# multiplefish/VPLines-SLAM

Measured on AMD Instinct MI355X. Metric: sliding-window BA solves/sec (10 KF, 200 pts + 80 lines, 5 iters), higher is better.
Workload: dtype f64

## Files before the change

vplines-slam_amd/csrc/ba_step.h:

```cpp
#pragma once
#include "ba_common.h"
#include "ba_solve.h"

namespace vpl {

constexpr int SCHUR_THREADS = 256;
constexpr int CHOL_THREADS = 256;
constexpr int BACK_THREADS = 256;

__device__ __forceinline__ void lds_ticket_wait(int* t, int seq) {
  while (__hip_atomic_load(t, __ATOMIC_RELAXED, __HIP_MEMORY_SCOPE_WORKGROUP) != seq) __builtin_amdgcn_s_sleep(1);
  __builtin_amdgcn_fence(__ATOMIC_ACQUIRE, "workgroup", "local");
}
__device__ __forceinline__ void lds_ticket_pass(int* t, int seq, int lane) {
  __builtin_amdgcn_fence(__ATOMIC_RELEASE, "workgroup", "local");
  if (lane == 0) __hip_atomic_store(t, seq + 1, __ATOMIC_RELAXED, __HIP_MEMORY_SCOPE_WORKGROUP);
}

__device__ __forceinline__ int compact2vis(int c, int s, int WS) {
  if (c < WS - 6) { const int v = 6 * s + c; return v < 66 ? v : -1; }
  if (c < WS) return 66 + (c - (WS - 6));
  return c < WS + 2 ? 72 + (c - WS) : -1;
}

// ... 287 lines not shown
      for (int b = 0; b < 4; ++b) if (b <= a) {
        A[t] = s4[a] * s4[b] * Hl[4 * a + b];
        if (a == b) A[t] += mu * d4[a] * d4[a];
        ++t;
      }
    bool ok = true;
    chol4(A, ok);
    if (!ok) flag[0] = 1;
    double us[4];
#pragma unroll
    for (int k = 0; k < 10; ++k) { lch[l * 10 + k] = A[k]; lC[l * 10 + k] = A[k]; }
#pragma unroll
    for (int a = 0; a < 4; ++a) {
      const double rd = 1.0 / A[tri(a, a)];
      lS[4 * l + a] = s4[a] * rd;
      us[a] = g4[a] / d4[a];
#pragma unroll
      for (int qd = 0; qd < 4; ++qd) if (qd < a) lC[l * 10 + tri(a, qd)] = A[tri(a, qd)] * rd;
    }
#pragma unroll
    for (int a = 0; a < 4; ++a) {
      double s2 = 0;
#pragma unroll
      for (int qd = 0; qd < 4; ++qd) if (qd >= a) s2 += A[tri(qd, a)] * us[qd];
      lE[4 * l + a] = s2;
    }
    {
      double xg[4];
#pragma unroll
      for (int a = 0; a < 4; ++a) {
        double s2 = (s4[a] / A[tri(a, a)]) * (g4[a] * d4[a] / s4[a]);
#pragma unroll
        for (int qd = 0; qd < 4; ++qd) if (qd < a) s2 -= (A[tri(a, qd)] / A[tri(a, a)]) * xg[qd];
        xg[a] = s2;
        lG[4 * l + a] = s2;
      }
    }
  }
  __syncthreads();
  for (int i = tid; i < CSQ_N; i += T) Cacc[i] = 0.0;
  for (int i = tid; i < NLT * 4 * 64; i += T) {
    const int ln = i & 63, v = (i >> 6) & 3, t = i >> 8;
    int ta = 0, tb = 0;
    tri_decode(t, ta, tb);
    const int ca = 16 * ta + (ln >> 4) + 4 * v, cb = 16 * tb + (ln & 15);
    int code = -1;
    if (ca >= cb && ca < WSv + 2 && cb < WSv) {
      const int a0 = compact2vis(ca, 0, WSv), b0 = compact2vis(cb, 0, WSv);
      const int step = (ca < WSv - 6 ? CSQ_LD : 0) + (cb < WSv - 6 ? 1 : 0);
      code = (a0 * CSQ_LD + b0) | step << 16;
    }
    ftab[i] = code;
  }
  __syncthreads();
  VPL_STAMP(B, w, 2);
  {
    const int m = lane & 15, kk = lane >> 4;
    const int wrow = lane < SK_WSTRIDE ? B.sk_wave[((size_t)w * 8 + wv) * SK_WSTRIDE + lane] : -1;
    const int nchunk = __builtin_amdgcn_readlane(wrow, 0);
    auto fetch = [&](int k) {
      int4 e = etab[k];
      e.x = __builtin_amdgcn_readfirstlane(e.x); e.y = __builtin_amdgcn_readfirstlane(e.y); e.z = __builtin_amdgcn_readfirstlane(e.z);
      return e;
    };
    v4d acc[NLT];
#pragma unroll
    for (int t = 0; t < NLT; ++t) acc[t] = v4d{0, 0, 0, 0};
    const double* Wp = B.Wp + (size_t)w * B.maxP * WS;
    const double* Wl = B.Wl + (size_t)w * B.maxL * 4 * WS;
    const double* gpv = B.gp + (size_t)w * B.maxP;
    const double* glv = B.gl + (size_t)w * B.maxL * 4;
    double wm[NTC], gm[NTC], em[NTC];
    int cl[NTC];
#pragma unroll
    for (int t = 0; t < NTC; ++t) {
      const int c = 16 * t + m;
      wm[t] = c < WSv ? 1.0 : 0.0;
      gm[t] = c == WSv ? 1.0 : 0.0;
      em[t] = c == WSv + 1 ? 1.0 : 0.0;
      cl[t] = c < WSv - 6 ? c : (c < WSv ? c + coff : WS - 1);
    }
    auto lm_id = [&](const int4 e) { return ((kk & 2 ? e.z : e.y) >> (16 * (kk & 1))) & 0xffff; };
    auto load_raw = [&](const int4 e, double (&raw)[NTC][4]) {
      const bool isl = (e.x & 32) != 0;
      const int idr = lm_id(e);
      const int id = idr != 0xffff ? idr : 0;
      if (isl) {
        const double* Wr = Wl + (unsigned)(id * 4 * WS);
#pragma unroll
        for (int t = 0; t < NTC; ++t)
#pragma unroll
          for (int qd = 0; qd < 4; ++qd) raw[t][qd] = Wr[(unsigned)(qd * WS + cl[t])];
      } else {
#pragma unroll
        for (int t = 0; t < NTC; ++t) raw[t][0] = Wp[(unsigned)(id * WS + cl[t])];
#pragma unroll
        for (int t = 0; t < NTC; ++t)
#pragma unroll
          for (int qd = 1; qd < 4; ++qd) raw[t][qd] = 0.0;
      }
    };
    auto transform = [&](const int4 e, const double (&raw)[NTC][4], double (&x)[NTC][4]) {
      const bool isl = (e.x & 32) != 0;
      const int idr = lm_id(e);
      const int id = idr != 0xffff ? idr : 0;
      const double pm = idr != 0xffff ? 1.0 : 0.0;
      if (isl) {
        const double* C = lC + id * 10;
        const double s0 = lS[4 * id] * pm, s1 = lS[4 * id + 1] * pm, s2 = lS[4 * id + 2] * pm, s3 = lS[4 * id + 3] * pm;
        const double c10 = C[1], c20 = C[3], c21 = C[4], c30 = C[6], c31 = C[7], c32 = C[8];
        double ev[4], gv[4];
#pragma unroll
        for (int a = 0; a < 4; ++a) { ev[a] = lE[4 * id + a] * pm; gv[a] = lG[4 * id + a] * pm; }
#pragma unroll
        for (int t = 0; t < NTC; ++t) {
          const double x0 = s0 * raw[t][0];
          const double x1 = s1 * raw[t][1] - c10 * x0;
          const double x2 = s2 * raw[t][2] - c20 * x0 - c21 * x1;
          const double x3 = s3 * raw[t][3] - c30 * x0 - c31 * x1 - c32 * x2;
          x[t][0] = x0 * wm[t] + gv[0] * gm[t] + ev[0] * em[t];
          x[t][1] = x1 * wm[t] + gv[1] * gm[t] + ev[1] * em[t];
          x[t][2] = x2 * wm[t] + gv[2] * gm[t] + ev[2] * em[t];
          x[t][3] = x3 * wm[t] + gv[3] * gm[t] + ev[3] * em[t];
        }
      } else {
        const double sp = pS[id] * pm, ep = pE[id] * pm, gq = pG[id] * pm;
#pragma unroll
        for (int t = 0; t < NTC; ++t) {
          x[t][0] = sp * raw[t][0] * wm[t] + gq * gm[t] + ep * em[t];
          x[t][1] = 0.0; x[t][2] = 0.0; x[t][3] = 0.0;
        }
      }
    };
#ifdef VPL_STAMPS
    long long st_flush = 0, st_wait = 0, st_xf = 0, st_mf = 0, st_ld = 0;
#endif
    auto flush = [&](int g, int seq) {
#ifdef VPL_STAMPS
      const long long tf0 = __builtin_readcyclecounter();
#endif
      const int s6 = 6 * (g & 15);
      int code[NLT * 4];
#pragma unroll
      for (int i = 0; i < NLT * 4; ++i) code[i] = ftab[i * 64 + lane];
      lds_ticket_wait(&tick[0], seq);
#ifdef VPL_STAMPS
      st_wait += __builtin_readcyclecounter() - tf0;
#endif
#pragma unroll
      for (int t = 0; t < NLT; ++t) {
        const double vals[4] = {acc[t].x, acc[t].y, acc[t].z, acc[t].w};
#pragma unroll
        for (int v = 0; v < 4; ++v) {
          const int c2 = code[4 * t + v];
          if (c2 >= 0) lds_add(&Cacc[(c2 & 0xffff) + s6 * (c2 >> 16)], vals[v]);
        }
        acc[t] = v4d{0, 0, 0, 0};
      }
      lds_ticket_pass(&tick[0], seq, lane);
#ifdef VPL_STAMPS
      st_flush += __builtin_readcyclecounter() - tf0;
#endif
    };
    int nent = 0;
#pragma unroll 1
    for (int ch = 0; ch < nchunk; ++ch) {
      const int k0 = __builtin_amdgcn_readlane(wrow, __builtin_amdgcn_readfirstlane(1 + 3 * ch));
      const int k1 = __builtin_amdgcn_readlane(wrow, __builtin_amdgcn_readfirstlane(2 + 3 * ch));
      const int seq = __builtin_amdgcn_readlane(wrow, __builtin_amdgcn_readfirstlane(3 + 3 * ch));
      nent += k1 - k0;
      if (MIXED && (fetch(k0).x & 64)) {
        SchurWide A;
        A.etab = etab; A.Wp = Wp; A.Wl = Wl; A.WS = WS; A.lC = lC; A.lS = lS; A.lE = lE; A.lG = lG; A.pS = pS; A.pE = pE; A.pG = pG;
        A.Cacc = Cacc; A.tick = tick;
        schur_wide_chunk(A, k0, k1, seq);
        continue;
      }
      double raw0[NTC][4], raw1[NTC][4], raw2[NTC][4];
      constexpr int NPF = 3;
      load_raw(fetch(k0), raw0);
      load_raw(fetch(min(k0 + 1, k1 - 1)), raw1);
      load_raw(fetch(min(k0 + 2, k1 - 1)), raw2);
      const int gcur = fetch(k0).x;
      auto step = [&](int k, double (&rw)[NTC][4]) {
        const int4 e = fetch(k);
#ifdef VPL_STAMPS
        const long long ts0 = __builtin_readcyclecounter();
#endif
        double x[NTC][4];
        transform(e, rw, x);
#ifdef VPL_STAMPS
        const long long ts1 = __builtin_readcyclecounter();
        st_xf += ts1 - ts0;
#endif
        load_raw(fetch(min(k + NPF, k1 - 1)), rw);
#ifdef VPL_STAMPS
        const long long ts2 = __builtin_readcyclecounter();
        st_ld += ts2 - ts1;
#endif
        const bool isl = (e.x & 32) != 0;
#pragma unroll
        for (int a = 0; a < 4; ++a) {
          if (a == 0 || isl) {
            int t = 0;
#pragma unroll
            for (int ta = 0; ta < NTC; ++ta)
#pragma unroll
              for (int tb = 0; tb <= ta; ++tb, ++t) acc[t] = __builtin_amdgcn_mfma_f64_16x16x4f64(x[ta][a], x[tb][a], acc[t], 0, 0, 0);
          }
        }
#ifdef VPL_STAMPS
        st_mf += __builtin_readcyclecounter() - ts2;
#endif
      };
#pragma unroll 1
      for (int kb = k0; kb < k1; kb += NPF) {
        step(kb, raw0);
        if (kb + 1 < k1) step(kb + 1, raw1);
        if (kb + 2 < k1) step(kb + 2, raw2);
      }
      flush(gcur, seq);
    }
#ifdef VPL_STAMPS
    if (lane == 0 && wv < 2) {
      long long* dg_ = B.dbg + (size_t)w * 64 + 30 + 6 * wv;
      dg_[0] = st_xf; dg_[1] = st_ld; dg_[2] = st_mf; dg_[3] = st_flush; dg_[4] = st_wait; dg_[5] = nent;
    }
#endif
  }
  __syncthreads();
  VPL_STAMP(B, w, 3);
  for (int b = tid; b < NV; b += T) qq += 2.0 * Cacc[(NV + 1) * CSQ_LD + b] * uc[vis2cam(b)];
  double* sacc = B.sacc + (size_t)w * SACC_N;
  for (int i = tid; i < SACC_N; i += T) {
    int a, b;
    tri_decode(i, a, b);
    sacc[i] = Cacc[a * CSQ_LD + b];
  }
  a1 = block_sum(a1, red);
  q = block_sum(q, red);
  qq = block_sum(qq, red);
  if (tid == 0) {
    tr->a1 = a1;
    tr->alpha = a1 / (q + qq);
    if (flag[0]) B.path[w] = 2;
  }
  VPL_STAMP(B, w, 4);
}

template <int NTC>
__global__ __launch_bounds__(SCHUR_THREADS, 2) void k_schur(DevBatch B) {
  extern __shared__ double sm[];
  if (blockIdx.x == 0 && threadIdx.x == 0) { B.ord_cnt[2 * ((B.ord_it + 1) & 1)] = 0; B.ord_cnt[2 * ((B.ord_it + 1) & 1) + 1] = 0; }
  schur_body<NTC>(B, ordered_window(B), sm);
}
__global__ __launch_bounds__(SCHUR_THREADS, 2) void k_schur_mixed(DevBatch B) {
  extern __shared__ double sm[];
  if (blockIdx.x == 0 && threadIdx.x == 0) { B.ord_cnt[2 * ((B.ord_it + 1) & 1)] = 0; B.ord_cnt[2 * ((B.ord_it + 1) & 1) + 1] = 0; }
  schur_body<3, true>(B, ordered_window(B), sm);
}
inline size_t schur_smem(int maxP, int maxL, int ntc = 5) {
  const int r1 = std::max(4 * maxP + 28 * maxL, (int)CSQ_N);
  const int maxKS = maxP / 4 + maxL + NF + 2;
  return (size_t)(r1 + 3 * maxP + 22 * maxL + 176 + 24) * sizeof(double) + (size_t)(8 + 4 * maxKS + ntc * (ntc + 1) / 2 * 256) * sizeof(int);
}

constexpr int DN = 90;
constexpr int DNT = 6;
constexpr int DNAP = DNT * (DNT + 1) / 2 * 256;
#ifdef VPL_CHOL_OCC3
constexpr int XLD = 66;
constexpr int CHOL_MIN_WAVES = 3;
#else
constexpr int XLD = 72;
constexpr int CHOL_MIN_WAVES = 2;
#endif
constexpr int XROWS_A = 36, XROWS_B = 48;

__device__ __forceinline__ int chain_frame(int ch, int b) { return ch == 0 ? 1 + b : 10 - b; }
__device__ __forceinline__ int chain_col(int ch, int b, int lane) {
  if (lane < 18) {
    const int ds = (b & 1) ? 9 : 0;
    const int f = chain_frame(ch, b);
    const int fr = (lane >= ds && lane < ds + 9) ? f : (ch == 0 ? f + 1 : f - 1);
    return 15 * fr + 6 + (lane < 9 ? lane : lane - 9);
  }
  if (ch == 0) {
    if (lane < 27) return 6 + (lane - 18);
    if (lane < 63) return 15 * ((lane - 27) / 6) + (lane - 27) % 6;
    return NC;
  }
  if (lane < 54) return 15 * (5 + (lane - 18) / 6) + (lane - 18) % 6;
  return lane == 54 ? NC : -1;
}
__device__ __forceinline__ int cam2dense(int c) {
  if (c < 0) return -1;
  if (c == NC) return DN;
  const int v = cam2vis(c);
  if (v >= 0) return v;
  if (c < 15) return 72 + (c - 6);
  return (c >= 81 && c < 90) ? c : -1;
}
__device__ __forceinline__ int dense2cam(int d) { return d < NV ? vis2cam(d) : (d < 81 ? 6 + (d - 72) : d); }
__device__ __forceinline__ int chain_dense(int ch, int lane) {
  if (lane < 18) {
    const bool s5 = ch == 0 ? lane < 9 : lane >= 9;
    return s5 ? 81 + (lane < 9 ? lane : lane - 9) : -1;
  }
  return cam2dense(chain_col(ch, 0, lane));
}

__device__ __forceinline__ void chol_body(const DevBatch& B, const int w, double* sm) {
  const int tid = threadIdx.x, T = CHOL_THREADS;
  const int lane = tid & 63, wv = ((tid >> 6) + ((blockIdx.x >> 8) & 1) * 2) & 3;
  TrState* tr = &B.tr[w];
  if (tr->status != 0 || tr->reuse != 0 || B.path[w] != 0) return;
  count_active(B, 1);
  constexpr int REG = (XROWS_A + XROWS_B) * XLD > DNAP ? (XROWS_A + XROWS_B) * XLD : DNAP;
  double* XA = sm;
  double* XBm = sm + XROWS_A * XLD;
  double* S = sm;
  double* scv = sm + REG;
  double* dgv = scv + 176;
  double* ycam = dgv + 176;
  double* yv = ycam + 176;
  double* isd = yv + 96;
  double* Linv = isd + 96;
  double* red = Linv + 256;
  int* flag = (int*)(red + 24);
  int* cdmap = flag + 8;
  double* rsL = (double*)(cdmap + 128);

  const size_t fb = (size_t)w * B.nfull;
  const double* gscale = B.scale + fb;
  const double* gdiag = B.diag + fb;
  const double* ggrad = B.grad + fb;
  double* ggn = B.gn + fb;
  const double* Hcc = B.Hcc + (size_t)w * NCP;
  const double* gc = B.gc + (size_t)w * NC;
  const double* sacc = B.sacc + (size_t)w * SACC_N;
  const double mu = tr->mu;
  for (int c = tid; c < 176; c += T) { scv[c] = c < NC ? gscale[c] : 0.0; dgv[c] = c < NC ? gdiag[c] : 1.0; ycam[c] = 0.0; }
  if (tid < 4) flag[tid] = 0;
  if (tid < 128) cdmap[tid] = chain_dense(tid >> 6, tid & 63);
  for (int i = tid; i < 3 * XLD; i += T) XBm[(XROWS_B - 3) * XLD + i] = 0.0;
  __syncthreads();
  VPL_STAMP(B, w, 8);

  double U[45];
#pragma unroll
  for (int i = 0; i < 45; ++i) U[i] = 0.0;
#define Xs(b, k) U[9 * (b) + (k)]
  if (wv < 2) {
    const int ch = wv, nblk = ch == 0 ? 4 : 5;
    double* Xout = ch == 0 ? XA : XBm;
    bool bad = false;
    auto load_strip = [&](int b, double (&raw)[9]) {
      const int col = chain_col(ch, b, lane);
      const int f = chain_frame(ch, b);
#pragma unroll
      for (int i = 0; i < 9; ++i) {
        const int r = 15 * f + 6 + i;
        raw[i] = 0.0;
        if (col == NC) raw[i] = gc[r];
        else if (col >= 0) raw[i] = Hcc[col > r ? tri(col, r) : tri(r, col)];
      }
    };
    double rawn[9];
    load_strip(0, rawn);
#pragma unroll
    for (int b = 0; b < 5; ++b) {
      if (b < nblk) {
        const int ds = (b & 1) ? 9 : 0, ns = 9 - ds;
        const int col = chain_col(ch, b, lane);
        const int f = chain_frame(ch, b);
        double R[9];
        {
          const double scol = col == NC ? 1.0 : (col >= 0 ? scv[col] : 0.0);
#pragma unroll
          for (int i = 0; i < 9; ++i) {
            const int r = 15 * f + 6 + i;
            R[i] = rawn[i] * (scv[r] * scol);
            if (col == r) R[i] += mu * dgv[r] * dgv[r];
          }
        }
        if (b + 1 < nblk) load_strip(b + 1, rawn);
        if (b > 0) {
          const bool fresh = lane >= ns && lane < ns + 9;
#pragma unroll
          for (int k = 0; k < 9; ++k) {
            const double xk = fresh ? 0.0 : Xs(b - 1, k);
#pragma unroll
            for (int i = 0; i < 9; ++i) R[i] -= readlane_f64(Xs(b - 1, k), ds + i) * xk;
          }
        }
        double piv[9];
#pragma unroll
        for (int k = 0; k < 9; ++k) {
          const double pk = readlane_f64(R[k], ds + k);
          piv[k] = pk;
          if (!(pk > 0.0)) bad = true;
          double rinv = __builtin_amdgcn_rcp(pk);
          rinv = fma(rinv, fma(-pk, rinv, 1.0), rinv);
          rinv = fma(rinv, fma(-pk, rinv, 1.0), rinv);
          const double fj = R[k] * rinv;
#pragma unroll
          for (int i = k + 1; i < 9; ++i) R[i] -= readlane_f64(R[i], ds + k) * fj;
        }
        const bool dcol = cam2dense(col) >= 0;
#pragma unroll
        for (int k = 0; k < 9; ++k) {
          double rs = __builtin_amdgcn_rsq(piv[k]);
          rs = rs * fma(-0.5 * piv[k] * rs, rs, 1.5);
          rs = rs * fma(-0.5 * piv[k] * rs, rs, 1.5);
          if (lane == 0) rsL[(5 * ch + b) * 9 + k] = rs;
          const double xv = R[k] * rs;
          Xs(b, k) = col >= 0 ? xv : 0.0;
          Xout[(9 * b + k) * XLD + lane] = dcol ? xv : 0.0;
        }
        __builtin_amdgcn_fence(__ATOMIC_RELEASE, "workgroup");
        if (lane == 0) __hip_atomic_store(&flag[1 + ch], b + 1, __ATOMIC_RELAXED, __HIP_MEMORY_SCOPE_WORKGROUP);
      }
    }
    if (bad && lane == 0) flag[0] = 1;
  } else {
    const int ch = wv - 2, nblk = ch == 0 ? 4 : 5;
    const double* Xin = ch == 0 ? XA : XBm;
    const int m = lane & 15, kk = lane >> 4;
    const int nks = (ch == 0 ? XROWS_A : XROWS_B) / 4;
    int have = 0;
    v4d pacc[10];
#pragma unroll
    for (int t = 0; t < 10; ++t) pacc[t] = v4d{0, 0, 0, 0};
    for (int ks = 0; ks < nks; ++ks) {
      const int need = min(nblk, (4 * ks + 3) / 9 + 1);
      while (have < need) {
        have = __hip_atomic_load(&flag[1 + ch], __ATOMIC_RELAXED, __HIP_MEMORY_SCOPE_WORKGROUP);
        if (have >= need) __builtin_amdgcn_fence(__ATOMIC_ACQUIRE, "workgroup");
      }
      const double* row = Xin + (4 * ks + kk) * XLD + m;
      const double x0 = row[0], x1 = row[16], x2 = row[32], x3 = row[48];
      pacc[0] = __builtin_amdgcn_mfma_f64_16x16x4f64(x0, x0, pacc[0], 0, 0, 0);
      pacc[1] = __builtin_amdgcn_mfma_f64_16x16x4f64(x1, x0, pacc[1], 0, 0, 0);
      pacc[2] = __builtin_amdgcn_mfma_f64_16x16x4f64(x1, x1, pacc[2], 0, 0, 0);
      pacc[3] = __builtin_amdgcn_mfma_f64_16x16x4f64(x2, x0, pacc[3], 0, 0, 0);
      pacc[4] = __builtin_amdgcn_mfma_f64_16x16x4f64(x2, x1, pacc[4], 0, 0, 0);
      pacc[5] = __builtin_amdgcn_mfma_f64_16x16x4f64(x2, x2, pacc[5], 0, 0, 0);
      pacc[6] = __builtin_amdgcn_mfma_f64_16x16x4f64(x3, x0, pacc[6], 0, 0, 0);
      pacc[7] = __builtin_amdgcn_mfma_f64_16x16x4f64(x3, x1, pacc[7], 0, 0, 0);
      pacc[8] = __builtin_amdgcn_mfma_f64_16x16x4f64(x3, x2, pacc[8], 0, 0, 0);
      pacc[9] = __builtin_amdgcn_mfma_f64_16x16x4f64(x3, x3, pacc[9], 0, 0, 0);
    }
#pragma unroll
    for (int t = 0; t < 10; ++t) { U[4 * t] = pacc[t].x; U[4 * t + 1] = pacc[t].y; U[4 * t + 2] = pacc[t].z; U[4 * t + 3] = pacc[t].w; }
  }
  __syncthreads();
  VPL_STAMP(B, w, 9);

  auto put = [&](int r, int c, double v) {
    S[tix(r, c)] = v;
    if ((r >> 4) == (c >> 4) && r != c) S[tix(c, r)] = v;
  };
  {
    constexpr int NVP = NV * (NV + 1) / 2;
    constexpr int NB1 = (NVP + CHOL_THREADS - 1) / CHOL_THREADS;
    constexpr int NB2 = (19 * 96 + CHOL_THREADS - 1) / CHOL_THREADS;
    double hh[NB1], ss[NB1], h2[NB2], s2[NB2];
    int rc1[NB1], rc2[NB2];
#pragma unroll
    for (int u = 0; u < NB1; ++u) {
      const int e = u * T + tid;
      hh[u] = 0.0; ss[u] = 0.0; rc1[u] = -1;
      if (e < NVP) {
        int vr, vc;
        tri_decode(e, vr, vc);
        rc1[u] = vr | vc << 8;
        hh[u] = Hcc[tri(vis2cam(vr), vis2cam(vc))];
        ss[u] = sacc[e];
      }
    }
#pragma unroll
    for (int u = 0; u < NB2; ++u) {
      const int idx = u * T + tid;
      const int i = idx / 96, dc = idx - 96 * i;
      const int dr = 72 + i;
      h2[u] = 0.0; s2[u] = 0.0; rc2[u] = -1;
      if (idx < 19 * 96 && dc <= dr && dc < DN) {
        rc2[u] = dr | dc << 8;
        const int c = dense2cam(dc);
        if (dr < DN) {
          const int r = dense2cam(dr);
          h2[u] = Hcc[r >= c ? tri(r, c) : tri(c, r)];
        } else {
          h2[u] = gc[c];
          if (dc < NV) s2[u] = sacc[tri(NV, dc)];
        }
      }
    }
    for (int i = tid; i < DNAP; i += T) S[i] = 0.0;
    __syncthreads();
    VPL_STAMP(B, w, 14);
#pragma unroll
    for (int u = 0; u < NB1; ++u)
      if (rc1[u] >= 0) {
        const int vr = rc1[u] & 255, vc = rc1[u] >> 8;
        const int r = vis2cam(vr), c = vis2cam(vc);
        double v = (hh[u] - ss[u]) * (scv[r] * scv[c]);
        if (r == c) v += mu * dgv[r] * dgv[r];
        put(vr, vc, v);
      }
#pragma unroll
    for (int u = 0; u < NB2; ++u)
      if (rc2[u] >= 0) {
        const int dr = rc2[u] & 255, dc = rc2[u] >> 8;
        const int c = dense2cam(dc);
        if (dr < DN) {
          const int r = dense2cam(dr);
          double v = h2[u] * (scv[r] * scv[c]);
          if (r == c) v += mu * dgv[r] * dgv[r];
          put(dr, dc, v);
        } else {
          put(DN, dc, (h2[u] - s2[u]) * scv[c]);
        }
      }
    if (tid < 6) S[tix(DN + tid, DN + tid)] = 1.0;
  }
  __syncthreads();
  VPL_STAMP(B, w, 15);
  auto in_both = [](int d) { return (d >= 30 && d < 36) || d >= 81; };
#pragma unroll 1
  for (int pass = 0; pass < 2; ++pass) {
    if ((wv == 2 && pass == 0) || wv == 3) {
      const int ch = wv - 2;
      const int m = lane & 15, kk = lane >> 4;
      int t = 0;
#pragma unroll
      for (int ta = 0; ta < 4; ++ta)
#pragma unroll
        for (int tb = 0; tb <= ta; ++tb, ++t) {
          const int j = 16 * tb + m, dj = cdmap[64 * ch + j];
#pragma unroll
          for (int v = 0; v < 4; ++v) {
            const int i = 16 * ta + kk + 4 * v;
            if (i < j) continue;
            const int di = cdmap[64 * ch + i];
            if (di < 0 || dj < 0) continue;
            if (ch == 1 && (in_both(di) && in_both(dj)) != (pass == 1)) continue;
            const int r = di > dj ? di : dj, c = di > dj ? dj : di;
            if (c >= DN) continue;
            const double val = U[4 * t + v];
            S[tix(r, c)] -= val;
            if ((r >> 4) == (c >> 4) && r != c) S[tix(c, r)] -= val;
          }
        }
    }
    __syncthreads();
  }
  VPL_STAMP(B, w, 10);

  {
    constexpr int NWV = CHOL_THREADS / 64;
    for (int K = 0; K < DNT; ++K) {
      auto rank_update = [&](int col, int I, int J0, int J1) {
        const int m = lane & 15, kk = lane >> 4;
        double* Ct = S + ((I * (I + 1) / 2 + col) << 8);
        v4d c;
        c.x = Ct[tsw(kk, m)]; c.y = Ct[tsw(kk + 4, m)]; c.z = Ct[tsw(kk + 8, m)]; c.w = Ct[tsw(kk + 12, m)];
        for (int J = J0; J < J1; ++J) {
          const double* Ai = S + ((I * (I + 1) / 2 + J) << 8);
          const double* Bk = S + ((col * (col + 1) / 2 + J) << 8);
#pragma unroll
          for (int ks = 0; ks < 4; ++ks) {
            const double av = -Ai[tsw(m, 4 * ks + kk)];
            const double bv = Bk[tsw(m, 4 * ks + kk)];
            c = __builtin_amdgcn_mfma_f64_16x16x4f64(av, bv, c, 0, 0, 0);
          }
        }
        Ct[tsw(kk, m)] = c.x; Ct[tsw(kk + 4, m)] = c.y; Ct[tsw(kk + 8, m)] = c.z; Ct[tsw(kk + 12, m)] = c.w;
      };
      if (wv == 0) {
        double* D = S + ((K * (K + 1) / 2 + K) << 8);
        const int r4 = lane >> 4, cc = lane & 15;
        double d[4], mm[4];
#pragma unroll
        for (int v = 0; v < 4; ++v) { d[v] = D[tsw(r4 + 4 * v, cc)]; mm[v] = (r4 + 4 * v == cc) ? 1.0 : 0.0; }
        const int ncol = min(16, DN - 16 * K);
        double pivc = 1.0;
        bool bad = false;
#define VPL_DSTEP(J) diag_tile_step<J>(d, mm, r4, cc, ncol, pivc, bad);
        VPL_DSTEP(0) VPL_DSTEP(1) VPL_DSTEP(2) VPL_DSTEP(3) VPL_DSTEP(4) VPL_DSTEP(5) VPL_DSTEP(6) VPL_DSTEP(7)
        VPL_DSTEP(8) VPL_DSTEP(9) VPL_DSTEP(10) VPL_DSTEP(11) VPL_DSTEP(12) VPL_DSTEP(13) VPL_DSTEP(14) VPL_DSTEP(15)
#undef VPL_DSTEP
        if (bad) {
          if (lane == 0) flag[0] = 1;
        } else {
          const double sq = sqrt(pivc);
          if (cc < ncol) {
#pragma unroll
            for (int v = 0; v < 4; ++v) {
              const int r = r4 + 4 * v;
              if (r > cc) D[tsw(r, cc)] = d[v] / sq;
              else if (r == cc) { const double id = 1.0 / sq; isd[16 * K + cc] = id; D[tsw(r, cc)] = 1.0 / id; }
            }
          }
          if (K < DNT - 1) {
            const double isq = 1.0 / sq;
#pragma unroll
            for (int v = 0; v < 4; ++v) {
              const int r = r4 + 4 * v;
              const double ir = __shfl(isq, r, 64);
              Linv[tsw(r, cc)] = cc <= r ? mm[v] * ir : 0.0;
            }
          }
        }
      } else if (K >= 1) {
        for (int I = K + 1 + (wv - 1); I < DNT; I += NWV - 1) rank_update(K, I, K - 1, K);
        if (K + 1 < DNT)
          for (int I = K + 1 + (wv - 1); I < DNT; I += NWV - 1) rank_update(K + 1, I, 0, K);
      }
      __syncthreads();
      if (flag[0]) break;
      for (int I = K + 1 + wv; I < DNT; I += NWV) {
        const int m = lane & 15, kk = lane >> 4;
        double* At = S + ((I * (I + 1) / 2 + K) << 8);
        v4d c = {0.0, 0.0, 0.0, 0.0};
        double av[4], bv[4];
#pragma unroll
        for (int ks = 0; ks < 4; ++ks) { av[ks] = At[tsw(m, 4 * ks + kk)]; bv[ks] = Linv[tsw(m, 4 * ks + kk)]; }
#pragma unroll
        for (int ks = 0; ks < 4; ++ks) c = __builtin_amdgcn_mfma_f64_16x16x4f64(av[ks], bv[ks], c, 0, 0, 0);
        At[tsw(kk, m)] = c.x; At[tsw(kk + 4, m)] = c.y; At[tsw(kk + 8, m)] = c.z; At[tsw(kk + 12, m)] = c.w;
        if (I == K + 1) {
          __builtin_amdgcn_fence(__ATOMIC_RELEASE, "workgroup");
          __builtin_amdgcn_wave_barrier();
          __builtin_amdgcn_fence(__ATOMIC_ACQUIRE, "workgroup");
          rank_update(K + 1, K + 1, K, K + 1);
        }
      }
      __syncthreads();
    }
  }
  __syncthreads();
  if (flag[0]) {
    if (tid == 0) B.path[w] = 2;
    return;
  }
  VPL_STAMP(B, w, 11);
  for (int c = tid; c < 96; c += T) yv[c] = c < DN ? S[tix(DN, c)] : 0.0;
  __syncthreads();
  for (int K = DNT - 1; K >= 0; --K) {
    const double* D = S + ((K * (K + 1) / 2 + K) << 8);
    if (wv == 0) {
      const int ncol = min(16, DN - 16 * K);
      double yl = lane < 16 ? yv[16 * K + lane] : 0.0;
      const double isdl = lane < ncol ? isd[16 * K + lane] : 0.0;
      double Lcol[16];
#pragma unroll
      for (int j = 0; j < 16; ++j) Lcol[j] = (lane < j && j < ncol) ? D[tsw(j, lane & 15)] : 0.0;
#pragma unroll
      for (int j = 15; j >= 0; --j) {
        if (j < ncol) {
          const double yj = readlane_f64(yl, j) * readlane_f64(isdl, j);
          if (lane < j) yl -= Lcol[j] * yj;
          if (lane == j) yl = yj;
        }
      }
      if (lane < ncol) yv[16 * K + lane] = yl;
    }
    __syncthreads();
    for (int c = tid; c < 16 * K; c += T) {
      const double* Lk = S + ((K * (K + 1) / 2 + (c >> 4)) << 8);
      double s2 = 0.0;
#pragma unroll
      for (int r = 0; r < 16; ++r) s2 += Lk[tsw(r, c & 15)] * yv[16 * K + r];
      yv[c] -= s2;
    }
    __syncthreads();
  }
  for (int d = tid; d < DN; d += T) ycam[dense2cam(d)] = yv[d];
  __syncthreads();
  VPL_STAMP(B, w, 12);
  if (wv < 2) {
    const int ch = wv, nblk = ch == 0 ? 4 : 5;
#pragma unroll
    for (int b = 4; b >= 0; --b) {
      if (b < nblk) {
        const int ds = (b & 1) ? 9 : 0;
        const int col = chain_col(ch, b, lane);
        const int f = chain_frame(ch, b);
        const bool pivl = lane >= ds && lane < ds + 9;
        const double cf = col == NC ? 1.0 : ((col < 0 || pivl) ? 0.0 : -ycam[col]);
        double t[9];
#pragma unroll
        for (int k = 0; k < 9; ++k) t[k] = wave_sum_dpp(Xs(b, k) * cf);
#pragma unroll
        for (int j = 8; j >= 0; --j) {
          const double yj = t[j] * rsL[(5 * ch + b) * 9 + j];
#pragma unroll
          for (int k = 0; k < j; ++k) t[k] -= readlane_f64(Xs(b, k), ds + j) * yj;
          t[j] = yj;
        }
        if (lane == 0) {
#pragma unroll
          for (int j = 0; j < 9; ++j) ycam[15 * f + 6 + j] = t[j];
        }
        __builtin_amdgcn_fence(__ATOMIC_RELEASE, "workgroup");
        __builtin_amdgcn_wave_barrier();
        __builtin_amdgcn_fence(__ATOMIC_ACQUIRE, "workgroup");
      }
    }
  }
  __syncthreads();
  double a2 = 0.0, a3 = 0.0;
  double* ycs = B.ycs + (size_t)w * 176;
  for (int c = tid; c < 176; c += T) {
    double u = 0.0;
    if (c < NC) {
      const double y = ycam[c];
      u = scv[c] * y;
      const double gnv = -dgv[c] * y;
      ggn[c] = gnv;
      a2 += gnv * gnv;
      a3 += ggrad[c] * gnv;
    }
    ycs[c] = u;
  }
  a2 = block_sum(a2, red);
  a3 = block_sum(a3, red);
  if (tid == 0) { B.sx[(size_t)w * 8] = a2; B.sx[(size_t)w * 8 + 1] = a3; }
  VPL_STAMP(B, w, 13);
}
#undef Xs
__global__ __launch_bounds__(CHOL_THREADS, CHOL_MIN_WAVES) void k_chol(DevBatch B) {
  extern __shared__ double sm[];
  chol_body(B, ordered_window(B), sm);
}
constexpr size_t CHOL_SMEM = (size_t)(((XROWS_A + XROWS_B) * XLD > DNAP ? (XROWS_A + XROWS_B) * XLD : DNAP) + 3 * 176 + 2 * 96 + 256 + 24 + 96) * sizeof(double) + (8 + 128) * sizeof(int);

__device__ __forceinline__ void back_body(const DevBatch& B, const int w, double* sm) {
  const int tid = threadIdx.x, T = BACK_THREADS;
  const int lane = tid & 63;
  TrState* tr = &B.tr[w];
  if (tr->status != 0) return;
  const int path = B.path[w];
  if (path != 0) {
    __syncthreads();
    if (tid == 0 && path == 2) B.path[w] = 0;
    return;
  }
  const int nP = B.nP[w], nL = B.nL[w];
  const int WS = B.WS;
  double* uc = sm;
  double* lrhs = uc + 176;
  double* lgn = lrhs + 4 * B.maxL;
  double* gdelta = lgn + B.nfull;
  double* red = gdelta + B.nfull;
  int* pSt = (int*)(red + 24);
  int* lSt = pSt + B.maxP;
  const size_t fb = (size_t)w * B.nfull;
  const double* gscale = B.scale + fb;
  const double* gdiag = B.diag + fb;
  const double* ggrad = B.grad + fb;
  double* ggn = B.gn + fb;
  const double* lch = B.lchol + (size_t)w * B.maxL * 10;
  const int LP = NC, LL = NC + B.maxP;
  const bool reuse0 = tr->reuse != 0;
  count_active(B, reuse0 ? 2 : 1);
  VPL_STAMP(B, w, 5);
  if (!reuse0) {
    const double mu = tr->mu;
    for (int p = tid; p < nP; p += T) pSt[p] = B.pt_start[(size_t)w * B.maxP + p];
    for (int l = tid; l < nL; l += T) lSt[l] = B.ln_start[(size_t)w * B.maxL + l];
    for (int c = tid; c < 176; c += T) uc[c] = c < NV ? B.ycs[(size_t)w * 176 + vis2cam(c)] : 0.0;
    for (int c = tid; c < NC; c += T) lgn[c] = ggn[c];
    __syncthreads();
    double a2 = 0.0, a3 = 0.0;
    {
      const int sub = lane & 7, grp = tid >> 3;
      const int nblk = WS / 6;
      constexpr int NPH = 4;
      for (int p0 = 0; p0 < nP; p0 += NPH * (T / 8)) {
        double wyv[NPH], sv[NPH], dv[NPH], hv[NPH], gv2[NPH], grv[NPH];
        size_t piv[NPH];
#pragma unroll
        for (int h = 0; h < NPH; ++h) {
          const int p = p0 + h * (T / 8) + grp;
          piv[h] = (size_t)w * B.maxP + (p < nP ? p : 0);
          wyv[h] = 0.0; sv[h] = dv[h] = 1.0; hv[h] = gv2[h] = grv[h] = 0.0;
          if (p < nP) {
            const int s0 = pSt[p];
            for (int blk = sub; blk < nblk; blk += 8) {
              const bool exb = blk == nblk - 1;
              const int vb = exb ? 66 : 6 * (s0 + blk);
              if (!exb && vb >= 66) continue;
              const double* Wr = B.Wp + piv[h] * WS + 6 * blk;
#pragma unroll
              for (int k = 0; k < 6; ++k) wyv[h] += Wr[k] * uc[vb + k];
            }
            if (sub == 0) {
              sv[h] = gscale[LP + p]; dv[h] = gdiag[LP + p]; hv[h] = B.Hpp[piv[h]]; gv2[h] = B.gp[piv[h]];
              grv[h] = ggrad[LP + p];
            }
          }
        }
#pragma unroll
        for (int h = 0; h < NPH; ++h) {
          const int p = p0 + h * (T / 8) + grp;
          double wy = wyv[h];
          wy += __shfl_xor(wy, 1, 64); wy += __shfl_xor(wy, 2, 64); wy += __shfl_xor(wy, 4, 64);
          if (p < nP && sub == 0) {
            const double s = sv[h], d = dv[h];
            const double Al = s * s * hv[h] + mu * d * d;
            const double y = s * (gv2[h] - wy) / Al;
            const double gnv = -d * y;
            ggn[LP + p] = gnv; lgn[LP + p] = gnv;
            a2 += gnv * gnv;
            a3 += grv[h] * gnv;
          }
        }
      }
      constexpr int NLH = 5;
      for (int r0 = 0; r0 < 4 * nL; r0 += NLH * (T / 8)) {
        double wyv[NLH], glv[NLH];
#pragma unroll
        for (int h = 0; h < NLH; ++h) {
          const int r = r0 + h * (T / 8) + grp, l = r >> 2, a = r & 3;
          wyv[h] = 0.0; glv[h] = 0.0;
          if (l < nL) {
            const size_t li = (size_t)w * B.maxL + l;
            const int s0 = lSt[l];
            for (int blk = sub; blk < nblk; blk += 8) {
              const bool exb = blk == nblk - 1;
              const int vb = exb ? 66 : 6 * (s0 + blk);
              if (!exb && vb >= 66) continue;
              const double* Wr = B.Wl + (li * 4 + a) * WS + 6 * blk;
#pragma unroll
              for (int k = 0; k < 6; ++k) wyv[h] += Wr[k] * uc[vb + k];
            }
            if (sub == 0) glv[h] = B.gl[li * 4 + a];
          }
        }
#pragma unroll
        for (int h = 0; h < NLH; ++h) {
          const int r = r0 + h * (T / 8) + grp;
          double wy = wyv[h];
          wy += __shfl_xor(wy, 1, 64); wy += __shfl_xor(wy, 2, 64); wy += __shfl_xor(wy, 4, 64);
          if (r < 4 * nL && sub == 0) lrhs[r] = gscale[LL + r] * (glv[h] - wy);
        }
      }
      __syncthreads();
      for (int l = tid; l < nL; l += T) {
        double C[10], t4[4], gd4[4], gr4[4];
#pragma unroll
        for (int k = 0; k < 10; ++k) C[k] = lch[l * 10 + k];
#pragma unroll
        for (int k = 0; k < 4; ++k) { gd4[k] = gdiag[LL + 4 * l + k]; gr4[k] = ggrad[LL + 4 * l + k]; }
#pragma unroll
        for (int k = 0; k < 4; ++k) t4[k] = lrhs[4 * l + k];
#pragma unroll
        for (int k = 0; k < 4; ++k) {
          double s2 = t4[k];
#pragma unroll
          for (int j = 0; j < 4; ++j) if (j < k) s2 -= C[tri(k, j)] * t4[j];
          t4[k] = s2 / C[tri(k, k)];
        }
#pragma unroll
        for (int k = 3; k >= 0; --k) {
          double s2 = t4[k];
#pragma unroll
          for (int j = 0; j < 4; ++j) if (j > k) s2 -= C[tri(j, k)] * t4[j];
          t4[k] = s2 / C[tri(k, k)];
        }
#pragma unroll
        for (int k = 0; k < 4; ++k) {
          const double gnv = -gd4[k] * t4[k];
          ggn[LL + 4 * l + k] = gnv; lgn[LL + 4 * l + k] = gnv;
          a2 += gnv * gnv;
          a3 += gr4[k] * gnv;
        }
      }
    }
    a2 = block_sum(a2, red);
    a3 = block_sum(a3, red);
    if (tid == 0) {
      tr->a2 = a2 + B.sx[(size_t)w * 8];
      tr->a3 = a3 + B.sx[(size_t)w * 8 + 1];
      tr->reuse = 1;
    }
    __syncthreads();
  }
  VPL_STAMP(B, w, 6);
  const double radius = tr->radius, alpha = tr->alpha, a1 = tr->a1, a2 = tr->a2, a3 = tr->a3, mu = tr->mu;
  const double gradient_norm = sqrt(a1), gauss_newton_norm = sqrt(a2);
  double c1, c2, dnorm;
  if (gauss_newton_norm <= radius) {
    c1 = 0.0; c2 = 1.0; dnorm = gauss_newton_norm;
  } else if (gradient_norm * alpha >= radius) {
    c1 = radius / gradient_norm; c2 = 0.0; dnorm = radius;
  } else {
    const double b_dot_a = -alpha * a3;
    const double a_sq = (alpha * gradient_norm) * (alpha * gradient_norm);
    const double bma = a_sq - 2 * b_dot_a + a2;
    const double c = b_dot_a - a_sq;
    const double d = sqrt(c * c + bma * (radius * radius - a_sq));
    const double beta = (c <= 0) ? (d - c) / bma : (radius * radius - a_sq) / (d + c);
    c1 = alpha * (1.0 - beta); c2 = beta;
    dnorm = sqrt(c1 * c1 * a1 - 2.0 * c1 * c2 * a3 + c2 * c2 * a2);
  }
  const double q_cauchy = a1 / alpha;
  const double sg = -c1 * a1 + c2 * a3;
  const double vHy = a1 + mu * a3;
  const double yHy = -a3 - mu * a2;
  const double sHs = c1 * c1 * q_cauchy + 2.0 * c1 * c2 * vHy + c2 * c2 * yHy;
  const double model_cost_change = -(sg + 0.5 * sHs);
  const bool valid = model_cost_change > 0.0;
  if (!valid) {
    if (tid == 0) {
      tr->step_valid = 0;
      tr->iter += 1;
      tr->num_invalid += 1;
      if (tr->num_invalid >= kMaxInvalid) { tr->status = 2; tr->iter -= 1; }
      else if (tr->iter >= B.opt.num_iterations) tr->status = 3;
      tr->mu *= kMuIncrease;
      tr->reuse = 0;
    }
    return;
  }
  const int nfull_used = NC + B.maxP + 4 * nL;
  for (int k = tid; k < nfull_used; k += T) {
    const bool live = k < NC || (k >= LP && k < LP + nP) || k >= LL;
    if (live) gdelta[k] = gscale[k] * (-c1 * ggrad[k] + c2 * (reuse0 ? ggn[k] : lgn[k])) / gdiag[k];
  }
  __syncthreads();
  double sn = 0.0, xn = 0.0;
  const bool ex_free = B.opt.estimate_extrinsic != 0;
  if (tid < NF + 1) {
    const bool isex = tid == NF;
    const double* x = isex ? B.ex + (size_t)w * 7 : B.pose + ((size_t)w * NF + tid) * 7;
    double* xc = isex ? B.ex_c + (size_t)w * 7 : B.pose_c + ((size_t)w * NF + tid) * 7;
    if (isex && !ex_free) {
      for (int k = 0; k < 7; ++k) xc[k] = x[k];
    } else {
      double out[7];
      pose_plus(x, gdelta + (isex ? 165 : 15 * tid), out);
      for (int k = 0; k < 7; ++k) { xc[k] = out[k]; sn += (x[k] - out[k]) * (x[k] - out[k]); xn += x[k] * x[k]; }
    }
  } else if (tid >= 64 && tid < 64 + NF) {
    const int f = tid - 64;
    const double* x = B.sb + ((size_t)w * NF + f) * 9;
    double* xc = B.sb_c + ((size_t)w * NF + f) * 9;
    for (int k = 0; k < 9; ++k) {
      const double d = gdelta[15 * f + 6 + k];
      xc[k] = x[k] + d;
      sn += d * d; xn += x[k] * x[k];
    }
  }
  for (int p = tid; p < nP; p += T) {
    const size_t pi = (size_t)w * B.maxP + p;
    const double d = gdelta[LP + p];
    B.invd_c[pi] = B.invd[pi] + d;
    sn += d * d; xn += B.invd[pi] * B.invd[pi];
  }
  for (int l = tid; l < nL; l += T) {
    const size_t li = (size_t)w * B.maxL + l;
    double out[4];
    line_orth_plus(B.orth + li * 4, gdelta + LL + 4 * l, out);
    for (int k = 0; k < 4; ++k) {
      const double x = B.orth[li * 4 + k];
      B.orth_c[li * 4 + k] = out[k];
      sn += (x - out[k]) * (x - out[k]); xn += x * x;
    }
    const Plk Lc_ = orth_to_plk(out);
    double* lwc = B.lw_c + li * 6;
    lwc[0] = Lc_.n.x; lwc[1] = Lc_.n.y; lwc[2] = Lc_.n.z; lwc[3] = Lc_.v.x; lwc[4] = Lc_.v.y; lwc[5] = Lc_.v.z;
  }
  sn = block_sum(sn, red);
  xn = block_sum(xn, red);
  VPL_STAMP(B, w, 7);
  if (tid == 0) {
    tr->dogleg_step_norm = dnorm;
    tr->model_cost_change = model_cost_change;
    tr->step_norm = sqrt(sn);
    tr->x_norm = sqrt(xn);
    tr->step_valid = 1;
    tr->num_invalid = 0;
  }
}
#ifndef VPL_BACK_WAVES
#define VPL_BACK_WAVES 2
#endif
__global__ __launch_bounds__(BACK_THREADS, VPL_BACK_WAVES) void k_back(DevBatch B) {
  extern __shared__ double sm[];
  back_body(B, ordered_window(B), sm);
}
inline size_t back_smem(int maxP, int maxL) {
  const int nfull = NC + maxP + 4 * maxL;
  return (size_t)(176 + 4 * maxL + 2 * nfull + 24) * sizeof(double) + (size_t)(maxP + maxL) * sizeof(int);
}

}
```

Measured before the change: 254,100.

## Stage chain products in LDS and fold subtraction into Schur assembly

The two chain waves now write their MFMA Gram products into packed triangular LDS buffers (PA, PB) instead of holding them in registers. Those products are subtracted while each S entry is assembled, which removes the separate two-pass scatter-subtract loop, its extra barriers, the full zeroing of S and the cdmap table. The global Hcc/sacc prefetch is moved ahead of the barrier so it overlaps the chain waves. In exchange, chol uses more shared memory, which may lower occupancy, and every assembled entry does extra index mapping and LDS reads.

```diff
diff --git a/vplines-slam_amd/csrc/ba_step.h b/vplines-slam_amd/csrc/ba_step.h
--- a/vplines-slam_amd/csrc/ba_step.h
+++ b/vplines-slam_amd/csrc/ba_step.h
@@ -613,13 +613,19 @@
   return (c >= 81 && c < 90) ? c : -1;
 }
 __device__ __forceinline__ int dense2cam(int d) { return d < NV ? vis2cam(d) : (d < 81 ? 6 + (d - 72) : d); }
-__device__ __forceinline__ int chain_dense(int ch, int lane) {
-  if (lane < 18) {
-    const bool s5 = ch == 0 ? lane < 9 : lane >= 9;
-    return s5 ? 81 + (lane < 9 ? lane : lane - 9) : -1;
-  }
-  return cam2dense(chain_col(ch, 0, lane));
-}
+__device__ __forceinline__ int dense_lane(int ch, int d) {
+  if (ch == 0) {
+    if (d < 36) return 27 + d;
+    if (d < 72) return -1;
+    return d < 81 ? 18 + (d - 72) : (d < DN ? d - 81 : 63);
+  }
+  if (d < 30 || (d >= 66 && d < 81)) return -1;
+  return d < 66 ? 18 + (d - 30) : (d < DN ? 9 + (d - 81) : 54);
+}
+constexpr int PB_LANE0 = 9, PB_LANES = 46;
+constexpr int PA_N = 64 * 65 / 2, PB_N = PB_LANES * (PB_LANES + 1) / 2;
+constexpr int CHOL_REG = (XROWS_A + XROWS_B) * XLD > DNAP + PB_N + PA_N ? (XROWS_A + XROWS_B) * XLD : DNAP + PB_N + PA_N;
+static_assert(DNAP + PB_N >= (XROWS_A + XROWS_B) * XLD, "chain A's product must not overlap the X rows");
 
 __device__ __forceinline__ void chol_body(const DevBatch& B, const int w, double* sm) {
   const int tid = threadIdx.x, T = CHOL_THREADS;
@@ -627,11 +633,12 @@
   TrState* tr = &B.tr[w];
   if (tr->status != 0 || tr->reuse != 0 || B.path[w] != 0) return;
   count_active(B, 1);
-  constexpr int REG = (XROWS_A + XROWS_B) * XLD > DNAP ? (XROWS_A + XROWS_B) * XLD : DNAP;
   double* XA = sm;
   double* XBm = sm + XROWS_A * XLD;
   double* S = sm;
-  double* scv = sm + REG;
+  double* PB = sm + DNAP;
+  double* PA = PB + PB_N;
+  double* scv = sm + CHOL_REG;
   double* dgv = scv + 176;
   double* ycam = dgv + 176;
   double* yv = ycam + 176;
@@ -639,8 +646,7 @@
   double* Linv = isd + 96;
   double* red = Linv + 256;
   int* flag = (int*)(red + 24);
-  int* cdmap = flag + 8;
-  double* rsL = (double*)(cdmap + 128);
+  double* rsL = (double*)(flag + 8);
 
   const size_t fb = (size_t)w * B.nfull;
   const double* gscale = B.scale + fb;
@@ -653,7 +659,6 @@
   const double mu = tr->mu;
   for (int c = tid; c < 176; c += T) { scv[c] = c < NC ? gscale[c] : 0.0; dgv[c] = c < NC ? gdiag[c] : 1.0; ycam[c] = 0.0; }
   if (tid < 4) flag[tid] = 0;
-  if (tid < 128) cdmap[tid] = chain_dense(tid >> 6, tid & 63);
   for (int i = tid; i < 3 * XLD; i += T) XBm[(XROWS_B - 3) * XLD + i] = 0.0;
   __syncthreads();
   VPL_STAMP(B, w, 8);
@@ -762,55 +767,78 @@
       pacc[8] = __builtin_amdgcn_mfma_f64_16x16x4f64(x3, x2, pacc[8], 0, 0, 0);
       pacc[9] = __builtin_amdgcn_mfma_f64_16x16x4f64(x3, x3, pacc[9], 0, 0, 0);
     }
-#pragma unroll
-    for (int t = 0; t < 10; ++t) { U[4 * t] = pacc[t].x; U[4 * t + 1] = pacc[t].y; U[4 * t + 2] = pacc[t].z; U[4 * t + 3] = pacc[t].w; }
+    double* P = ch == 0 ? PA : PB;
+    const int l0 = ch == 0 ? 0 : PB_LANE0, nl = ch == 0 ? 64 : PB_LANES;
+    int t = 0;
+#pragma unroll
+    for (int ta = 0; ta < 4; ++ta)
+#pragma unroll
+      for (int tb = 0; tb <= ta; ++tb, ++t) {
+        const double pv[4] = {pacc[t].x, pacc[t].y, pacc[t].z, pacc[t].w};
+        const int j = 16 * tb + m - l0;
+#pragma unroll
+        for (int v = 0; v < 4; ++v) {
+          const int i = 16 * ta + kk + 4 * v - l0;
+          if (i >= j && j >= 0 && i < nl) P[tri(i, j)] = pv[v];
+        }
+      }
+  }
+
+  constexpr int NVP = NV * (NV + 1) / 2;
+  constexpr int NB1 = (NVP + CHOL_THREADS - 1) / CHOL_THREADS;
+  constexpr int NB2 = (19 * 96 + CHOL_THREADS - 1) / CHOL_THREADS;
+  double hh[NB1], ss[NB1], h2[NB2], s2[NB2];
+  int rc1[NB1], rc2[NB2];
+#pragma unroll
+  for (int u = 0; u < NB1; ++u) {
+    const int e = u * T + tid;
+    hh[u] = 0.0; ss[u] = 0.0; rc1[u] = -1;
+    if (e < NVP) {
+      int vr, vc;
+      tri_decode(e, vr, vc);
+      rc1[u] = vr | vc << 8;
+      hh[u] = Hcc[tri(vis2cam(vr), vis2cam(vc))];
+      ss[u] = sacc[e];
+    }
+  }
+#pragma unroll
+  for (int u = 0; u < NB2; ++u) {
+    const int idx = u * T + tid;
+    const int i = idx / 96, dc = idx - 96 * i;
+    const int dr = 72 + i;
+    h2[u] = 0.0; s2[u] = 0.0; rc2[u] = -1;
+    if (idx < 19 * 96 && dc <= dr && dc < DN) {
+      rc2[u] = dr | dc << 8;
+      const int c = dense2cam(dc);
+      if (dr < DN) {
+        const int r = dense2cam(dr);
+        h2[u] = Hcc[r >= c ? tri(r, c) : tri(c, r)];
+      } else {
+        h2[u] = gc[c];
+        if (dc < NV) s2[u] = sacc[tri(NV, dc)];
+      }
+    }
   }
   __syncthreads();
   VPL_STAMP(B, w, 9);
-
-  auto put = [&](int r, int c, double v) {
-    S[tix(r, c)] = v;
-    if ((r >> 4) == (c >> 4) && r != c) S[tix(c, r)] = v;
-  };
   {
-    constexpr int NVP = NV * (NV + 1) / 2;
-    constexpr int NB1 = (NVP + CHOL_THREADS - 1) / CHOL_THREADS;
-    constexpr int NB2 = (19 * 96 + CHOL_THREADS - 1) / CHOL_THREADS;
-    double hh[NB1], ss[NB1], h2[NB2], s2[NB2];
-    int rc1[NB1], rc2[NB2];
-#pragma unroll
-    for (int u = 0; u < NB1; ++u) {
-      const int e = u * T + tid;
-      hh[u] = 0.0; ss[u] = 0.0; rc1[u] = -1;
-      if (e < NVP) {
-        int vr, vc;
-        tri_decode(e, vr, vc);
-        rc1[u] = vr | vc << 8;
-        hh[u] = Hcc[tri(vis2cam(vr), vis2cam(vc))];
-        ss[u] = sacc[e];
-      }
-    }
-#pragma unroll
-    for (int u = 0; u < NB2; ++u) {
-      const int idx = u * T + tid;
-      const int i = idx / 96, dc = idx - 96 * i;
-      const int dr = 72 + i;
-      h2[u] = 0.0; s2[u] = 0.0; rc2[u] = -1;
-      if (idx < 19 * 96 && dc <= dr && dc < DN) {
-        rc2[u] = dr | dc << 8;
-        const int c = dense2cam(dc);
-        if (dr < DN) {
-          const int r = dense2cam(dr);
-          h2[u] = Hcc[r >= c ? tri(r, c) : tri(c, r)];
-        } else {
-          h2[u] = gc[c];
-          if (dc < NV) s2[u] = sacc[tri(NV, dc)];
-        }
-      }
-    }
-    for (int i = tid; i < DNAP; i += T) S[i] = 0.0;
-    __syncthreads();
+    for (int e = tid; e < 6 * 256; e += T) {
+      const int r = 80 + ((e >> 4) & 15), c = 16 * (e >> 8) + (e & 15);
+      if ((r > DN || c > DN) && r != c) S[tix(r, c)] = 0.0;
+    }
+    if (tid < 6) S[tix(DN + tid, DN + tid)] = 1.0;
     VPL_STAMP(B, w, 14);
+    auto chains = [&](int r, int c, double v) {
+      const int a0 = dense_lane(0, r), a1 = dense_lane(0, c);
+      if (a0 >= 0 && a1 >= 0) v -= PA[a0 > a1 ? tri(a0, a1) : tri(a1, a0)];
+      const int b0 = dense_lane(1, r) - PB_LANE0, b1 = dense_lane(1, c) - PB_LANE0;
+      if (b0 >= 0 && b1 >= 0) v -= PB[b0 > b1 ? tri(b0, b1) : tri(b1, b0)];
+      return v;
+    };
+    auto put = [&](int r, int c, double v) {
+      S[tix(r, c)] = v;
+      if ((r >> 4) == (c >> 4) && r != c) S[tix(c, r)] = v;
+    };
 #pragma unroll
     for (int u = 0; u < NB1; ++u)
       if (rc1[u] >= 0) {
@@ -818,7 +846,7 @@
         const int r = vis2cam(vr), c = vis2cam(vc);
         double v = (hh[u] - ss[u]) * (scv[r] * scv[c]);
         if (r == c) v += mu * dgv[r] * dgv[r];
-        put(vr, vc, v);
+        put(vr, vc, chains(vr, vc, v));
       }
 #pragma unroll
     for (int u = 0; u < NB2; ++u)
@@ -829,44 +857,14 @@
           const int r = dense2cam(dr);
           double v = h2[u] * (scv[r] * scv[c]);
           if (r == c) v += mu * dgv[r] * dgv[r];
-          put(dr, dc, v);
+          put(dr, dc, chains(dr, dc, v));
         } else {
-          put(DN, dc, (h2[u] - s2[u]) * scv[c]);
-        }
-      }
-    if (tid < 6) S[tix(DN + tid, DN + tid)] = 1.0;
+          put(DN, dc, chains(DN, dc, (h2[u] - s2[u]) * scv[c]));
+        }
+      }
+    VPL_STAMP(B, w, 15);
   }
   __syncthreads();
-  VPL_STAMP(B, w, 15);
-  auto in_both = [](int d) { return (d >= 30 && d < 36) || d >= 81; };
-#pragma unroll 1
-  for (int pass = 0; pass < 2; ++pass) {
-    if ((wv == 2 && pass == 0) || wv == 3) {
-      const int ch = wv - 2;
-      const int m = lane & 15, kk = lane >> 4;
-      int t = 0;
-#pragma unroll
-      for (int ta = 0; ta < 4; ++ta)
-#pragma unroll
-        for (int tb = 0; tb <= ta; ++tb, ++t) {
-          const int j = 16 * tb + m, dj = cdmap[64 * ch + j];
-#pragma unroll
-          for (int v = 0; v < 4; ++v) {
-            const int i = 16 * ta + kk + 4 * v;
-            if (i < j) continue;
-            const int di = cdmap[64 * ch + i];
-            if (di < 0 || dj < 0) continue;
-            if (ch == 1 && (in_both(di) && in_both(dj)) != (pass == 1)) continue;
-            const int r = di > dj ? di : dj, c = di > dj ? dj : di;
-            if (c >= DN) continue;
-            const double val = U[4 * t + v];
-            S[tix(r, c)] -= val;
-            if ((r >> 4) == (c >> 4) && r != c) S[tix(c, r)] -= val;
-          }
-        }
-    }
-    __syncthreads();
-  }
   VPL_STAMP(B, w, 10);
 
   {
@@ -1046,7 +1044,7 @@
   extern __shared__ double sm[];
   chol_body(B, ordered_window(B), sm);
 }
-constexpr size_t CHOL_SMEM = (size_t)(((XROWS_A + XROWS_B) * XLD > DNAP ? (XROWS_A + XROWS_B) * XLD : DNAP) + 3 * 176 + 2 * 96 + 256 + 24 + 96) * sizeof(double) + (8 + 128) * sizeof(int);
+constexpr size_t CHOL_SMEM = (size_t)(CHOL_REG + 3 * 176 + 2 * 96 + 256 + 24 + 96) * sizeof(double) + 8 * sizeof(int);
 
 __device__ __forceinline__ void back_body(const DevBatch& B, const int w, double* sm) {
   const int tid = threadIdx.x, T = BACK_THREADS;
```

Measured after the change: 256,300 (median of 6 runs). No clear change (+0.9%).
